# ZenHKD/ocr-vi-invoice

Hardware: AMD Instinct MI355X
Metric: invoice images/sec end-to-end (det+rec) (higher is better)
Workload: dtype f16x2

## Files before the change

### include/ocrvi.h

```cpp
#ifndef OCRVI_H
#define OCRVI_H

#include <stddef.h>
#include <stdint.h>

#ifdef __cplusplus
extern "C" {
#endif

#define OCRVI_OK 0
#define OCRVI_EINVAL (-1)
#define OCRVI_EHIP (-2)
#define OCRVI_ENOMEM (-3)
#define OCRVI_EBLOB (-4)
#define OCRVI_ERANGE (-5)

typedef enum { OCRVI_F32 = 0, OCRVI_BF16 = 1, OCRVI_F16 = 2, OCRVI_F16X2 = 3 } ocrvi_dtype;

const char* ocrvi_last_error(void);
int ocrvi_abi_version(void);

typedef struct ocrvi_det ocrvi_det;

typedef struct {
// ... 137 lines not shown

#define OCRVI_DB_TARGET_GT 0
#define OCRVI_DB_TARGET_MASK 1
#define OCRVI_DB_TARGET_THRESH 2
#define OCRVI_DB_TARGET_JOB 8
#define OCRVI_DB_TARGET_MAX_SIDE 16384
int ocrvi_db_target_jobs(const int32_t* sizes, const float* xy, const int32_t* poly_offsets, const int32_t* image_offsets, int n_images,
                         double shrink_ratio, int want_thresh, int32_t* jobs, int cap_jobs, int32_t* points, int cap_points, int32_t* n_jobs,
                         int32_t* n_points, int32_t* overflow, int threads);
int ocrvi_db_target_maps(int device, const int32_t* jobs, int n_jobs, const int32_t* points, int n_points, const int32_t* rows, int n, int S,
                         float thresh_max, float* gt, float* mask, float* thresh_map, float* thresh_mask, void* stream);
int ocrvi_resize_normalize_pad_pages(int device, const int64_t* pages, const int32_t* rows, int n, int S, float* out, void* stream);

#define OCRVI_DET_EVAL_RECORD_BYTES 104
#define OCRVI_DET_EVAL_TP 0
#define OCRVI_DET_EVAL_FP 1
#define OCRVI_DET_EVAL_FN 2
#define OCRVI_DET_EVAL_POSITIVES 3
#define OCRVI_DET_EVAL_NEGATIVES 4
#define OCRVI_DET_EVAL_K 5
#define OCRVI_DET_EVAL_POS_BCE 6
#define OCRVI_DET_EVAL_TOPK_BCE 7
#define OCRVI_DET_EVAL_DICE_INTER 8
#define OCRVI_DET_EVAL_PRED_MASK 9
#define OCRVI_DET_EVAL_GT_MASK 10
#define OCRVI_DET_EVAL_L1_NUM 11
#define OCRVI_DET_EVAL_THRESH_MASK 12
int ocrvi_det_eval_workspace_bytes(int N, int H, int W, size_t* bytes);
int ocrvi_det_eval(int device, const float* binary, const float* thresh, const float* thresh_binary, const float* bin_logits,
                   const float* gt, const float* mask, const float* thresh_map, const float* thresh_mask, int N, int H, int W,
                   double negative_ratio, void* record, void* workspace, size_t workspace_bytes, void* stream);

#define OCRVI_CTC_LOSS_MAX_TARGET 1024
int ocrvi_ctc_loss(int device, const float* log_probs, int T, int B, int C, const int32_t* targets, int Lmax, const int32_t* target_lengths,
                   const int32_t* input_lengths, int blank, double* nll, void* stream);

#define OCRVI_EDIT_DISTANCE_MAX_LEN 2048
int ocrvi_edit_distance(int device, const int32_t* pred_ids, int T, const int32_t* pred_lens, const int32_t* gt_ids, int G,
                        const int32_t* gt_lens, int B, int32_t* dist, void* stream);

int ocrvi_test_offset_conv(int device, int dtype, const float* x, const float* weight_host, const float* bias_host, int N, int C, int H, int W,
                           int stride, float* out, int iters, float* avg_ms);
int ocrvi_test_deform_conv(int device, int dtype, const float* x, const float* offset, const float* mask,
                           const float* weight_host, const float* bias_host, int N, int C, int H, int W, int Co,
                           int stride, int relu, float* out, int iters, float* avg_ms);
int ocrvi_test_deform_conv_res(int device, int dtype, const float* x, const float* offset, const float* mask,
                               const float* weight_host, const float* bias_host, const float* res, int N, int C, int H, int W, int Co,
                               int stride, int relu, float* out, int iters, float* avg_ms);
int ocrvi_test_conv(int device, int dtype, const float* x, const float* weight_host, const float* bias_host,
                    int N, int C, int H, int W, int Co, int ksize, int sh, int sw, int groups, int act, float* out,
                    int iters, float* avg_ms);
int ocrvi_test_conv_res(int device, int dtype, const float* x, const float* weight_host, const float* bias_host, const float* res, int N,
                        int C, int H, int W, int Co, int ksize, int res_mode, int act, float* out, int iters, float* avg_ms);
int ocrvi_test_bneck_tail(int device, const float* t1, const float* identity, const float* w2_host, const float* b2_host,
                          const float* w3_host, const float* b3_host, const float* w1_host, const float* b1_host, int N, int H, int W,
                          int no_phase_c, float* y_out, float* t1n_out, int iters, float* avg_ms);
int ocrvi_test_db_tail(int device, int dtype, const float* x, const float* dc1_w_bin_host, const float* dc1_b_bin_host,
                       const float* dc1_w_thr_host, const float* dc1_b_thr_host, const float* dc2_w_bin_host, const float* dc2_b_bin_host,
                       const float* dc2_w_thr_host, const float* dc2_b_thr_host, int N, int OH, int OW, int groups, int binary_only,
                       float* out, float* out2, int iters, float* avg_ms);
int ocrvi_test_gemm(int device, int dtype, const float* a, const float* weight_host, const float* bias_host, const float* res, int M,
                    int K, int N, int act, int res_post, int out_f32, float* out, int iters, float* avg_ms);
int ocrvi_test_gemm_raw(int device, int dtype, const float* a, const float* weight_host, const float* bias_host, const float* res, int M,
                        int K, int N, int act, int res_post, int out_f32, void* out_raw, float* out);
int ocrvi_test_ring_plan(int dtype, int amode, int M, int K, int N, int out_f32, int has_res, int n_cu, int32_t plan[8]);
int ocrvi_test_stem_pool(int device, int dtype, const float* x, const float* weight_host, const float* bias_host, int N, int H, int W, int fused,
                         float* out, int iters, float* avg_ms);
int ocrvi_test_attention(int device, int dtype, const float* qkv, int B, int N, int heads, float* out, int iters,
                         float* avg_ms);

int ocrvi_test_mlp(int device, int dtype, float* x, const float* ln_g_host, const float* ln_b_host, const float* w1_host, const float* b1_host,
                   const float* w2_host, const float* b2_host, const float* next_g_host, const float* next_b_host, int want_xn, int M, int D,
                   float* xn_out, int iters, float* avg_ms);
int ocrvi_test_mlp_raw(int device, int dtype, float* x, const float* ln_g_host, const float* ln_b_host, const float* w1_host, const float* b1_host,
                       const float* w2_host, const float* b2_host, const float* next_g_host, const float* next_b_host, int M, int D, void* xn_raw,
                       float* xn_out, int iters, float* avg_ms);
int ocrvi_test_pack_f16x2(const float* src, size_t n, void* dst, float* wscale);

int ocrvi_test_layernorm(int device, int dtype, const float* x, int x_f32, int out_f32, const float* gamma_host, const float* beta_host,
                         int rows, int D, float* out);
int ocrvi_test_frm_vertical(int device, int dtype, const float* kv, const float* vq_host, int B, int H, int W, int D, float* out);
int ocrvi_test_asf(int device, int dtype, const float* p2, const float* p3, const float* p4, const float* p5, const float* w_host,
                   const float* b_host, int N, int H, int W, float* out);
int ocrvi_test_maxpool(int device, int dtype, const float* x, int N, int C, int H, int W, float* out);
int ocrvi_test_db_maps(int device, const float* bin_logits, const float* thresh_logits, float k, float* binary, float* thresh,
                       float* thresh_binary, size_t n);
int ocrvi_test_ctc_logsoftmax(int device, const float* logits, int ld, int B, int T, int C, float* log_probs, int32_t* argmax_ids);

int ocrvi_prof_enable(int on);
int ocrvi_prof_reset(void);
int ocrvi_prof_report(char* buf, size_t cap);

#ifdef __cplusplus
}
#endif
#endif
```

### ocr_vi_invoice_amd/_lib.py

```python
from __future__ import annotations

import ctypes as C
import os
from typing import Optional

_HERE = os.path.dirname(os.path.abspath(__file__))
LIB_PATH = os.environ.get("OCRVI_LIB") or os.path.join(_HERE, "lib", "libocrvi.so")

OCRVI_F32, OCRVI_BF16, OCRVI_F16, OCRVI_F16X2 = 0, 1, 2, 3
DTYPES = {"f32": OCRVI_F32, "fp32": OCRVI_F32, "float32": OCRVI_F32, "bf16": OCRVI_BF16, "bfloat16": OCRVI_BF16,
          "f16": OCRVI_F16, "fp16": OCRVI_F16, "float16": OCRVI_F16,
          "f16x2": OCRVI_F16X2}
ABI_VERSION = 5

EXPORTS = [
    "ocrvi_last_error", "ocrvi_abi_version",
    "ocrvi_det_create", "ocrvi_det_destroy", "ocrvi_det_workspace_bytes", "ocrvi_det_forward", "ocrvi_det_debug_features",
    "ocrvi_rec_create", "ocrvi_rec_destroy", "ocrvi_rec_workspace_bytes", "ocrvi_rec_forward", "ocrvi_rec_debug_features",
    "ocrvi_ctc_greedy", "ocrvi_normalize_u8", "ocrvi_resize_u8", "ocrvi_crop_resize_normalize", "ocrvi_db_postprocess", "ocrvi_db_boxes_batch",
    "ocrvi_unclip_polygon", "ocrvi_db_components_workspace_bytes", "ocrvi_db_components", "ocrvi_db_boxes_batch_sparse",
    "ocrvi_test_deform_conv", "ocrvi_test_offset_conv", "ocrvi_test_conv", "ocrvi_test_gemm", "ocrvi_test_attention", "ocrvi_test_mlp", "ocrvi_test_stem_pool", "ocrvi_test_pack_f16x2",
    "ocrvi_prof_enable", "ocrvi_prof_reset", "ocrvi_prof_report",
    "ocrvi_det_status", "ocrvi_rec_status", "ocrvi_range_reset", "ocrvi_range_flag",
    "ocrvi_resize_normalize_pages", "ocrvi_crop_resize_normalize_pages", "ocrvi_db_boxes_pages",
    "ocrvi_det_binary_workspace_bytes", "ocrvi_det_forward_binary",
    "ocrvi_four_point_transform", "ocrvi_warp_perspective_u8", "ocrvi_warp_perspective_pages",
    "ocrvi_test_layernorm", "ocrvi_test_frm_vertical", "ocrvi_test_asf", "ocrvi_test_maxpool", "ocrvi_test_db_maps", "ocrvi_test_ctc_logsoftmax",
    "ocrvi_det_eval_workspace_bytes", "ocrvi_det_eval", "ocrvi_ctc_loss", "ocrvi_edit_distance",
    "ocrvi_test_deform_conv_res",
    "ocrvi_enhance_init", "ocrvi_enhance_tables", "ocrvi_enhance_workspace_bytes", "ocrvi_enhance_u8",
    "ocrvi_rgb_to_lab_u8", "ocrvi_lab_to_rgb_u8", "ocrvi_clahe_lab_u8", "ocrvi_nlm_lab_u8", "ocrvi_sharpen_u8",
    "ocrvi_min_area_quads", "ocrvi_quad_crops", "ocrvi_crop_quad_resize_normalize_pages", "ocrvi_crop_quad_resize_normalize",
    "ocrvi_jpeg_info", "ocrvi_jpeg_parse", "ocrvi_jpeg_table_entry", "ocrvi_jpeg_decode_pages",
    "ocrvi_test_conv_res", "ocrvi_test_db_tail",
    "ocrvi_db_target_jobs", "ocrvi_db_target_maps", "ocrvi_resize_normalize_pad_pages",
    "ocrvi_test_mlp_raw",
    "ocrvi_test_bneck_tail",
    "ocrvi_jpeg_quant_tables", "ocrvi_jpeg_encode_header", "ocrvi_jpeg_encode_sizes", "ocrvi_jpeg_encode_table_entry", "ocrvi_jpeg_encode_pages",
    "ocrvi_test_gemm_raw", "ocrvi_test_ring_plan",
]
PAGE_ENTRY = 4
DET_EVAL_RECORD_BYTES = 104
DET_EVAL_INT_SLOTS = ("tp", "fp", "fn", "positive_count", "negatives", "negative_count")
DET_EVAL_F64_SLOTS = ("pos_bce", "topk_bce", "dice_inter", "pred_mask", "gt_mask", "l1_num", "thresh_mask")
CTC_LOSS_MAX_TARGET = 1024
EDIT_DISTANCE_MAX_LEN = 2048
CLAHE_WORKSPACE_BYTES = 16384
ENHANCE_MIN_SIDE = 16
DB_TARGET_GT, DB_TARGET_MASK, DB_TARGET_THRESH = 0, 1, 2
DB_TARGET_JOB = 8
DB_TARGET_MAX_SIDE = 16384
JPEG_ENTRY = 64
JPEG_ENC_ENTRY = 64
JPEG_HEADER_MAX = 640


class DetCfg(C.Structure):
    _fields_ = [("dtype", C.c_int32), ("k", C.c_float), ("max_batch", C.c_int32), ("backbone", C.c_int32), ("no_dcn", C.c_int32),
                ("reserved", C.c_int32 * 3)]


class RecCfg(C.Structure):
    _fields_ = [("dtype", C.c_int32), ("dims", C.c_int32 * 3), ("num_blocks", C.c_int32 * 3), ("num_local", C.c_int32 * 3),
                ("num_classes", C.c_int32), ("blank_id", C.c_int32), ("reserved", C.c_int32 * 4)]


class JpegInfo(C.Structure):
    _fields_ = [("width", C.c_int32), ("height", C.c_int32), ("components", C.c_int32), ("h_samp", C.c_int32 * 3), ("v_samp", C.c_int32 * 3),
                ("restart_interval", C.c_int32), ("orientation", C.c_int32), ("out_height", C.c_int32), ("out_width", C.c_int32),
                ("reserved", C.c_int32), ("blocks", C.c_int64), ("stream_bytes", C.c_uint64), ("workspace_bytes", C.c_uint64),
                ("quant", (C.c_uint16 * 64) * 3), ("reason", C.c_char * 160)]


_lib: Optional[C.CDLL] = None


def load() -> C.CDLL:
    global _lib
    if _lib is not None:
        return _lib
    if not os.path.exists(LIB_PATH):
        raise RuntimeError(
            f"libocrvi.so not found at {LIB_PATH}: build it with `python -c 'import __graft_entry__ as g; g.build()'` "
            "(or `make -C ocr_vi_invoice_amd/csrc`).  There is no CPU fallback for the product path.")
    import torch
    lib = C.CDLL(LIB_PATH)
    vp, i32, f32p, i32p, sz = C.c_void_p, C.c_int, C.c_void_p, C.c_void_p, C.c_size_t
    lib.ocrvi_last_error.restype = C.c_char_p
    lib.ocrvi_last_error.argtypes = []
    lib.ocrvi_abi_version.restype = i32
    lib.ocrvi_det_create.argtypes = [i32, vp, sz, C.POINTER(DetCfg), C.POINTER(vp)]
    lib.ocrvi_det_destroy.argtypes = [vp]
    lib.ocrvi_det_destroy.restype = None
    lib.ocrvi_det_workspace_bytes.argtypes = [vp, i32, i32, i32, C.POINTER(sz)]
    lib.ocrvi_det_forward.argtypes = [vp, f32p, i32, i32, i32, f32p, f32p, f32p, f32p, f32p, vp, sz, vp]
    lib.ocrvi_det_binary_workspace_bytes.argtypes = [vp, i32, i32, i32, C.POINTER(sz)]
    lib.ocrvi_det_forward_binary.argtypes = [vp, f32p, i32, i32, i32, f32p, vp, sz, vp]
    lib.ocrvi_det_debug_features.argtypes = [vp, i32, i32, i32, f32p, f32p, f32p, f32p, f32p, vp, sz, vp]
    lib.ocrvi_rec_create.argtypes = [i32, vp, sz, C.POINTER(RecCfg), C.POINTER(vp)]
    lib.ocrvi_rec_destroy.argtypes = [vp]
    lib.ocrvi_rec_destroy.restype = None
    lib.ocrvi_rec_workspace_bytes.argtypes = [vp, i32, i32, i32, C.POINTER(sz)]
    lib.ocrvi_rec_forward.argtypes = [vp, f32p, i32, i32, i32, f32p, i32p, i32p, i32p, vp, sz, vp]
    lib.ocrvi_rec_debug_features.argtypes = [vp, i32, i32, i32, f32p, f32p, vp, sz, vp]
    lib.ocrvi_ctc_greedy.argtypes = [i32, f32p, i32, i32, i32, i32, i32p, i32p, i32p, vp]
    lib.ocrvi_normalize_u8.argtypes = [i32, vp, i32, i32, i32, f32p, vp]
    lib.ocrvi_resize_u8.argtypes = [i32, vp, i32, i32, vp, i32, i32, vp]
    lib.ocrvi_crop_resize_normalize.argtypes = [i32, vp, i32, i32, i32, i32p, i32, i32, i32, f32p, vp]
    lib.ocrvi_db_postprocess.argtypes = [vp, i32, i32, C.c_float, C.c_float, i32, C.c_float, C.c_float, vp, i32, vp, vp, i32, C.POINTER(i32)]
    lib.ocrvi_db_components_workspace_bytes.argtypes = [i32, i32, i32]
    lib.ocrvi_db_components_workspace_bytes.restype = sz
    lib.ocrvi_db_components.argtypes = [i32, vp, i32, i32, i32, C.c_float, vp, vp, vp, i32, vp, vp, C.c_longlong, vp, vp]
    lib.ocrvi_db_boxes_batch_sparse.argtypes = [vp, vp, vp, i32, vp, vp, C.c_longlong, i32, i32, i32, C.c_float, i32, C.c_float, C.c_float,
                                                C.c_double, C.c_double, i32, i32, i32, vp, vp, i32, vp, i32, vp]
    lib.ocrvi_unclip_polygon.argtypes = [vp, i32, C.c_double, vp, i32, C.POINTER(i32)]
    lib.ocrvi_db_boxes_batch.argtypes = [vp, i32, i32, i32, C.c_float, C.c_float, i32, C.c_float, C.c_float, C.c_double, C.c_double, i32, i32, i32,
                                         vp, vp, i32, vp, i32]
    lib.ocrvi_resize_normalize_pages.argtypes = [i32, vp, i32, i32, i32, f32p, vp]
    lib.ocrvi_crop_resize_normalize_pages.argtypes = [i32, vp, i32, i32p, i32, i32, i32, f32p, vp]
    lib.ocrvi_four_point_transform.argtypes = [vp, vp, vp, i32p, i32p]
    lib.ocrvi_warp_perspective_u8.argtypes = [i32, vp, i32, i32, vp, vp, i32, i32, vp]
    lib.ocrvi_warp_perspective_pages.argtypes = [i32, vp, vp, vp, i32, vp]
    lib.ocrvi_db_boxes_pages.argtypes = [vp, i32, i32, i32, C.c_float, C.c_float, i32, C.c_float, C.c_float, vp, vp, vp, vp, vp,
                                         vp, i32, vp, vp, vp, i32, vp, vp, i32]
    lib.ocrvi_test_deform_conv.argtypes = [i32, i32, f32p, f32p, f32p, vp, vp, i32, i32, i32, i32, i32, i32, i32, f32p, i32,
                                           C.POINTER(C.c_float)]
    lib.ocrvi_test_deform_conv_res.argtypes = [i32, i32, f32p, f32p, f32p, vp, vp, f32p, i32, i32, i32, i32, i32, i32, i32, f32p, i32,
                                               C.POINTER(C.c_float)]
    lib.ocrvi_test_offset_conv.argtypes = [i32, i32, f32p, vp, vp, i32, i32, i32, i32, i32, f32p, i32, C.POINTER(C.c_float)]
    lib.ocrvi_test_conv.argtypes = [i32, i32, f32p, vp, vp, i32, i32, i32, i32, i32, i32, i32, i32, i32, i32, f32p, i32,
                                    C.POINTER(C.c_float)]
    lib.ocrvi_test_conv_res.argtypes = [i32, i32, f32p, vp, vp, f32p, i32, i32, i32, i32, i32, i32, i32, i32, f32p, i32, C.POINTER(C.c_float)]
    lib.ocrvi_test_bneck_tail.argtypes = [i32, f32p, f32p, vp, vp, vp, vp, vp, vp, i32, i32, i32, i32, f32p, f32p, i32, C.POINTER(C.c_float)]
    lib.ocrvi_test_db_tail.argtypes = [i32, i32, f32p, vp, vp, vp, vp, vp, vp, vp, vp, i32, i32, i32, i32, i32, f32p, f32p, i32,
                                       C.POINTER(C.c_float)]
    lib.ocrvi_test_gemm.argtypes = [i32, i32, f32p, vp, vp, f32p, i32, i32, i32, i32, i32, i32, f32p, i32, C.POINTER(C.c_float)]
    lib.ocrvi_test_gemm_raw.argtypes = [i32, i32, f32p, vp, vp, f32p, i32, i32, i32, i32, i32, i32, vp, f32p]
    lib.ocrvi_test_ring_plan.argtypes = [i32, i32, i32, i32, i32, i32, i32, i32, C.POINTER(C.c_int32)]
    lib.ocrvi_test_stem_pool.argtypes = [i32, i32, f32p, vp, vp, i32, i32, i32, i32, f32p, i32, C.POINTER(C.c_float)]
    lib.ocrvi_test_attention.argtypes = [i32, i32, f32p, i32, i32, i32, f32p, i32, C.POINTER(C.c_float)]
    lib.ocrvi_test_mlp.argtypes = [i32, i32, f32p, vp, vp, vp, vp, vp, vp, vp, vp, i32, i32, i32, f32p, i32, C.POINTER(C.c_float)]
    lib.ocrvi_test_mlp_raw.argtypes = [i32, i32, f32p, vp, vp, vp, vp, vp, vp, vp, vp, i32, i32, vp, f32p, i32, C.POINTER(C.c_float)]
    lib.ocrvi_test_pack_f16x2.argtypes = [f32p, sz, vp, C.POINTER(C.c_float)]
    lib.ocrvi_test_layernorm.argtypes = [i32, i32, f32p, i32, i32, vp, vp, i32, i32, f32p]
    lib.ocrvi_test_frm_vertical.argtypes = [i32, i32, f32p, vp, i32, i32, i32, i32, f32p]
    lib.ocrvi_test_asf.argtypes = [i32, i32, f32p, f32p, f32p, f32p, vp, vp, i32, i32, i32, f32p]
    lib.ocrvi_test_maxpool.argtypes = [i32, i32, f32p, i32, i32, i32, i32, f32p]
    lib.ocrvi_test_db_maps.argtypes = [i32, f32p, f32p, C.c_float, f32p, f32p, f32p, sz]
    lib.ocrvi_test_ctc_logsoftmax.argtypes = [i32, f32p, i32, i32, i32, i32, f32p, i32p]
    lib.ocrvi_det_eval_workspace_bytes.argtypes = [i32, i32, i32, C.POINTER(sz)]
    lib.ocrvi_det_eval.argtypes = [i32, f32p, f32p, f32p, f32p, f32p, f32p, f32p, f32p, i32, i32, i32, C.c_double, vp, vp, sz, vp]
    lib.ocrvi_ctc_loss.argtypes = [i32, f32p, i32, i32, i32, i32p, i32, i32p, i32p, i32, vp, vp]
    lib.ocrvi_edit_distance.argtypes = [i32, i32p, i32, i32p, i32p, i32, i32p, i32, i32p, vp]
    lib.ocrvi_enhance_init.argtypes = [i32]
    lib.ocrvi_enhance_tables.argtypes = [vp, sz, C.POINTER(sz)]
    lib.ocrvi_enhance_workspace_bytes.argtypes = [i32, i32, C.POINTER(sz)]
    lib.ocrvi_enhance_u8.argtypes = [i32, vp, i32, i32, vp, vp, sz, vp]
    for name in ("ocrvi_rgb_to_lab_u8", "ocrvi_lab_to_rgb_u8", "ocrvi_nlm_lab_u8", "ocrvi_sharpen_u8"):
        getattr(lib, name).argtypes = [i32, vp, i32, i32, vp, vp]
    lib.ocrvi_clahe_lab_u8.argtypes = [i32, vp, i32, i32, vp, vp, sz, vp]
    lib.ocrvi_min_area_quads.argtypes = [vp, vp, i32, vp, vp]
    lib.ocrvi_quad_crops.argtypes = [vp, vp, i32, vp, vp, vp, vp]
    lib.ocrvi_crop_quad_resize_normalize_pages.argtypes = [i32, vp, i32, i32p, vp, i32, i32, i32, f32p, vp]
    lib.ocrvi_crop_quad_resize_normalize.argtypes = [i32, vp, i32, i32, i32, i32p, vp, i32, i32, i32, f32p, vp]
    lib.ocrvi_jpeg_info.argtypes = [vp, sz, C.POINTER(JpegInfo)]
    lib.ocrvi_jpeg_parse.argtypes = [vp, sz, vp, sz, C.POINTER(sz)]
    lib.ocrvi_jpeg_table_entry.argtypes = [C.POINTER(JpegInfo), sz, C.c_int64, C.c_int64, C.c_int64, C.c_int64, vp]
    lib.ocrvi_jpeg_decode_pages.argtypes = [i32, vp, vp, i32, vp, vp, sz, vp]
    lib.ocrvi_jpeg_quant_tables.argtypes = [i32, vp, vp]
    lib.ocrvi_jpeg_encode_header.argtypes = [i32, i32, i32, i32, i32, vp, sz, C.POINTER(sz)]
    lib.ocrvi_jpeg_encode_sizes.argtypes = [i32, i32, i32, i32, C.POINTER(C.c_int64), C.POINTER(C.c_uint64), C.POINTER(C.c_uint64), vp]
    lib.ocrvi_jpeg_encode_table_entry.argtypes = [i32, i32, i32, i32, i32, C.c_int64, C.c_int64, C.c_int64, C.c_int64, C.c_int64, vp]
    lib.ocrvi_jpeg_encode_pages.argtypes = [i32, vp, vp, i32, vp, vp, vp, sz, vp]
    lib.ocrvi_db_target_jobs.argtypes = [vp, vp, vp, vp, i32, C.c_double, i32, vp, i32, vp, i32, C.POINTER(C.c_int32), C.POINTER(C.c_int32),
                                         C.POINTER(C.c_int32), i32]
    lib.ocrvi_db_target_maps.argtypes = [i32, vp, i32, vp, i32, vp, i32, i32, C.c_float, f32p, f32p, f32p, f32p, vp]
    lib.ocrvi_resize_normalize_pad_pages.argtypes = [i32, vp, vp, i32, i32, f32p, vp]
    lib.ocrvi_det_status.argtypes = [vp]
    lib.ocrvi_rec_status.argtypes = [vp]
    lib.ocrvi_range_reset.argtypes = [i32, vp]
    lib.ocrvi_range_flag.argtypes = [i32, C.POINTER(i32)]
    lib.ocrvi_prof_enable.argtypes = [i32]
    lib.ocrvi_prof_reset.argtypes = []
    lib.ocrvi_prof_report.argtypes = [C.c_char_p, sz]
    for name in EXPORTS:
# ... 45 lines not shown
```

### ocr_vi_invoice_amd/csrc/conv_launch.h

```cpp
#pragma once
#include <stdlib.h>
#include <string.h>

#include <algorithm>

#include "conv_gemm.h"
#include "gemm_ring.h"
#include "gconv32.h"
#include "dcn_pipe.h"
#include "offs_conv.h"
#include "conv3_halo.h"

namespace ocrvi {

template <typename T, int AMODE, int BM, int BN, int WM, int WN>
static int launch_tile(const ConvParams& p, hipStream_t stream) {
    constexpr int smem = (BM + BN) * 128;
    const int total = cdiv(p.M, BM) * (p.Np / BN);
    hipLaunchKernelGGL((conv_gemm_kernel<T, AMODE, BM, BN, WM, WN, 0>), dim3(total, p.groups), dim3(256), smem, stream, p);
    OCRVI_HIP(hipGetLastError());
    return OCRVI_OK;
}

template <typename T, int BM, int NW, int SPS, bool F32O, bool C3, int BN, int ACT>
// ... 140 lines not shown
    }
}

template <typename T>
int launch_conv(const ConvParams& p_in, int amode, hipStream_t stream) {
    constexpr int EPC = TypeInfo<T>::EPC, BKE = 8 * EPC;
    ConvParams p = p_in;
    OCRVI_CHECK(p.M > 0 && p.M < (1 << 23) && p.OW > 0 && p.OH > 0, OCRVI_EINVAL, "conv: M=%d outside (0, 2^23)", p.M);
    p.mg_ow = ((1ull << 40) / (unsigned long long)p.OW) + 1;
    p.mg_oh = ((1ull << 40) / (unsigned long long)p.OH) + 1;
    p.identity_pix = (amode == AM_CONV1 && p.SH == 1 && p.SW == 1 && p.PH == 0 && p.PW == 0 && p.H == p.OH && p.W == p.OW &&
                      p.store_mode == ST_NHWC && p.res_mode != RES_UP2) ? 1 : 0;
    {
        const int osz = (p.out_f32 || sizeof(T) == 4) ? 4 : 2, per = 16 / osz;
        p.epi_lds = (p.store_mode == ST_NHWC && p.res_mode != RES_UP2 && p.N_g % per == 0 && p.ldo % per == 0 &&
                     p.out_coff % per == 0 && ((uintptr_t)p.out & 15) == 0) ? 1 : 0;
        const bool raw32 = IsF32<T>::value || (p.out_f32 && p.res_f32);
        p.res_in_store = (p.epi_lds && p.res_mode == RES_SAME && osz == 4 && raw32 && p.act == ACT_NONE &&
                          p.ldr % 4 == 0 && ((uintptr_t)p.res & 15) == 0) ? 1 : 0;
    }
    OCRVI_CHECK(p.x && p.w && p.out, OCRVI_EINVAL, "conv: null operand");
    OCRVI_CHECK(p.M > 0 && p.M == p.n_img * p.OH * p.OW, OCRVI_EINVAL, "conv: M=%d != %d*%d*%d", p.M, p.n_img, p.OH, p.OW);
    OCRVI_CHECK(p.Kp > 0 && p.Kp % BKE == 0, OCRVI_EINVAL, "conv: Kp=%d not a multiple of %d", p.Kp, BKE);
    OCRVI_CHECK(p.groups >= 1 && p.N_g >= 1, OCRVI_EINVAL, "conv: bad groups/N");
    OCRVI_CHECK((size_t)p.M * (size_t)(p.ldo > 32 ? p.ldo : 32) < ((size_t)1 << 40), OCRVI_EINVAL, "conv: output too large");
    if (p.store_mode == ST_DB_TAIL) {
        OCRVI_CHECK(amode == AM_CONV1 && p.shuffle_co == 64 && p.N_g == 256 && p.Np == 256 && p.out2 && p.offs && p.bias && p.groups == 2,
                    OCRVI_EINVAL, "db-tail deconv: needs 2 groups of 4x64 columns, both logit maps and the second-deconv weights");
    } else if (p.store_mode == ST_DB_BIN) {
        OCRVI_CHECK(amode == AM_CONV1 && p.shuffle_co == 64 && p.N_g == 256 && p.Np == 256 && p.offs && p.bias && p.groups == 1 && p.out_f32,
                    OCRVI_EINVAL, "db-bin deconv: needs one group of 4x64 columns, the fp32 binary map and the second-deconv weights");
    } else if (p.store_mode != ST_DCN_OFFS) {
        OCRVI_CHECK(p.N_g % 4 == 0 && p.ldo % 4 == 0 && p.out_coff % 4 == 0, OCRVI_EINVAL,
                    "conv: N_g=%d ldo=%d coff=%d must be multiples of 4", p.N_g, p.ldo, p.out_coff);
    } else {
        OCRVI_CHECK(p.bias && p.N_g <= 32 && p.groups == 1, OCRVI_EINVAL, "dcn offset conv: needs bias, N<=32");
    }
    if (p.res_mode != RES_NONE) OCRVI_CHECK(p.res && p.ldr % 4 == 0, OCRVI_EINVAL, "conv: residual missing / ldr%%4");
    if (p.res_mode == RES_UP2) OCRVI_CHECK(p.OH % 2 == 0 && p.OW % 2 == 0, OCRVI_EINVAL, "conv: RES_UP2 needs even OH/OW");
    if (p.store_mode == ST_SHUFFLE2)
        OCRVI_CHECK(p.shuffle_co > 0 && p.shuffle_co % 4 == 0 && p.N_g == 4 * p.shuffle_co, OCRVI_EINVAL, "conv: bad pixel-shuffle N");
    if (amode == AM_ROWS) {
        OCRVI_CHECK(p.groups == 1 && p.Hp >= (p.OH - 1) * p.SH + p.KH && p.Wp >= (p.OW - 1) * p.SW + 8 && p.Wp % 2 == 0 &&
                        p.Kp >= p.KH * 32 && (p.SW * 4) % EPC == 0,
                    OCRVI_EINVAL, "rows-mode conv: padded input %dx%d too small for %dx%d out", p.Hp, p.Wp, p.OH, p.OW);
        return launch_mode<T, AM_ROWS>(p, stream);
    }
    OCRVI_CHECK(p.Cin_g % EPC == 0 && p.Cin % EPC == 0 && p.cin_off % EPC == 0 && p.cin_off + p.groups * p.Cin_g <= p.Cin,
                OCRVI_EINVAL, "conv: channel counts Cin=%d Cin_g=%d off=%d must be multiples of %d", p.Cin, p.Cin_g, p.cin_off, EPC);
    const int ks = amode == AM_CONV1 ? 1 : 3;
    OCRVI_CHECK(p.Kp >= ks * ks * p.Cin_g, OCRVI_EINVAL, "conv: Kp=%d < %d", p.Kp, ks * ks * p.Cin_g);
    OCRVI_CHECK((p.OH - 1) * p.SH - p.PH + ks - 1 < p.H + ks && (p.OW - 1) * p.SW - p.PW + ks - 1 < p.W + ks, OCRVI_EINVAL,
                "conv: output %dx%d inconsistent with input %dx%d", p.OH, p.OW, p.H, p.W);
    if constexpr (sizeof(T) == 2) {
        if (gconv32_eligible(p, amode, 2)) return launch_gconv32<T>(p, stream);
    }
    if (offs_conv_eligible(p, amode, TypeInfo<T>::dtype)) return launch_offs_conv<T>(p, stream);
    if constexpr (IsSplit<T>::value) {
        if (conv3_halo_eligible(p, amode, TypeInfo<T>::dtype)) return launch_conv3_halo<T>(p, stream);
    }
    OCRVI_CHECK(!p.w_quartets, OCRVI_EINVAL,
                "conv3x3: weights are packed for the halo kernel but this call is not eligible for it (stride / epilogue / alignment)");
    if (gemm_ring_eligible(p, amode, TypeInfo<T>::dtype)) return launch_gemm_ring<T>(p, amode, stream);
    switch (amode) {
        case AM_CONV1: return launch_mode<T, AM_CONV1>(p, stream);
        case AM_CONV3: return launch_mode<T, AM_CONV3>(p, stream);
        case AM_DCN:
            OCRVI_CHECK(p.offs && p.Cin_g % BKE == 0 && p.groups == 1, OCRVI_EINVAL, "dcn: needs offsets and Cin %% %d == 0", BKE);
            if (dcn_pipe_eligible(p, TypeInfo<T>::dtype)) return launch_dcn_pipe<T>(p, stream);
            OCRVI_CHECK(!dcn_pipe_packing(TypeInfo<T>::dtype, p.Cin_g), OCRVI_EINVAL,
                        "dcn: weights are packed for the pipelined kernel but this call is not eligible for it (epilogue / alignment)");
            return launch_mode<T, AM_DCN>(p, stream);
        default: break;
    }
    set_error("conv: unknown A mode %d", amode);
    return OCRVI_EINVAL;
}

}
```

### ocr_vi_invoice_amd/csrc/gconv32.h

```cpp
#pragma once
#include "conv_gemm.h"

namespace ocrvi {

constexpr int GC_PS = 96;
constexpr int GC_TH = 4;
constexpr int GC_NBX = 5;

template <typename T, bool F32O>
__global__ __launch_bounds__(256, 2) void gconv32_kernel(const ConvParams p, int TH, int nbx, int bands_y, int bands_x, unsigned hw_magic) {
    constexpr int PS = GC_PS, MB = (GC_TH * GC_NBX + 3) / 4;
    extern __shared__ __attribute__((aligned(16))) char smem[];
    const int tid = threadIdx.x, lane = tid & 63, wave = tid >> 6;
    const int lr = lane & 15, g4 = lane >> 4;
    const int TW = 16 * nbx, HW = TW + 2, HH = TH + 2;
    char* const halo = smem;
    char* const wl = smem + HH * HW * PS;
    const int gp = blockIdx.y;
    const int ntile = p.n_img * bands_y * bands_x;
    const T* const Xg = (const T*)p.x + p.cin_off + gp * 32;
    constexpr int HPASS = ((GC_TH + 2) * (16 * GC_NBX + 2) * 4 + 255) / 256, WPASS = (32 * 36 + 255) / 256;
    uint4 hv[HPASS];
    const int htotal = HH * HW * 4;
    auto tile_origin = [&](int t, int& img, int& y0, int& x0) {
        const int bx = t % bands_x;
        t /= bands_x;
        const int by = t % bands_y;
        img = t / bands_y;
        y0 = by * TH;
        x0 = bx * TW;
    };
    auto fetch = [&](int t) {
        int img, y0, x0;
        tile_origin(t, img, y0, x0);
        const T* X = Xg + (size_t)img * p.H * p.W * p.Cin;
#pragma unroll
        for (int k = 0; k < HPASS; ++k) {
            const int i = min(tid + 256 * k, htotal - 1);
            const int pix = i >> 2, c = i & 3;
            const int hy = (int)(((unsigned)pix * hw_magic) >> 16), hx = pix - hy * HW;
            const int iy = min(max(y0 + hy - 1, 0), p.H - 1), ix = min(max(x0 + hx - 1, 0), p.W - 1);
            hv[k] = *(const uint4*)(X + ((size_t)iy * p.W + ix) * p.Cin + c * 8);
        }
    };
    auto stage = [&](int t) {
        int img, y0, x0;
        tile_origin(t, img, y0, x0);
#pragma unroll
        for (int k = 0; k < HPASS; ++k) {
            const int i = tid + 256 * k;
            if (i < htotal) {
                const int pix = i >> 2, c = i & 3;
                const int hy = (int)(((unsigned)pix * hw_magic) >> 16), hx = pix - hy * HW;
                const int iy = y0 + hy - 1, ix = x0 + hx - 1;
// ... 61 lines not shown
            const int r = tap / 3, s = tap - r * 3;
            uint4 wf[2];
#pragma unroll
            for (int nb = 0; nb < 2; ++nb) wf[nb] = *(const uint4*)(wl + (tap * 32 + wrow[nb]) * PS + g4 * 16);
#pragma unroll
            for (int m = 0; m < MB; ++m) {
                if (wave + 4 * m < nblk) {
                    const uint4 xf = *(const uint4*)(halo + aoff[m] + (r * HW + s) * PS);
                    Mma<T>::half(wf[0], xf, acc[m][0]);
                    Mma<T>::half(wf[1], xf, acc[m][1]);
                }
            }
        }
        __syncthreads();
        if (next < ntile) stage(next);
        int img, y0, x0;
        tile_origin(tile, img, y0, x0);
#pragma unroll
        for (int m = 0; m < MB; ++m) {
            const int mb = wave + 4 * m, ty = mb / nbx, tb = mb - ty * nbx;
            const int y = y0 + ty, x = x0 + tb * 16 + lr;
            if (mb >= nblk || y >= p.H || x >= p.W) continue;
            const size_t pix = ((size_t)img * p.H + y) * p.W + x;
            float v[2][4];
#pragma unroll
            for (int nb = 0; nb < 2; ++nb) {
                const int ch = gp * 32 + (F32O ? nb * 16 + 4 * g4 : 8 * g4 + 4 * nb);
                v[nb][0] = acc[m][nb][0] + bias_r[nb].x; v[nb][1] = acc[m][nb][1] + bias_r[nb].y;
                v[nb][2] = acc[m][nb][2] + bias_r[nb].z; v[nb][3] = acc[m][nb][3] + bias_r[nb].w;
                if (p.res_post) activate(v[nb]);
                if (F32O && p.res_mode == RES_SAME) {
                    const float4 rv = *(const float4*)((const float*)p.res + pix * p.ldr + ch);
                    v[nb][0] += rv.x; v[nb][1] += rv.y; v[nb][2] += rv.z; v[nb][3] += rv.w;
                }
                if (!p.res_post) activate(v[nb]);
                if (F32O) *(float4*)((float*)p.out + pix * p.ldo + p.out_coff + ch) = make_float4(v[nb][0], v[nb][1], v[nb][2], v[nb][3]);
            }
            if (!F32O) {
                union { T e[8]; uint4 u; } pk;
#pragma unroll
                for (int e = 0; e < 4; ++e) {
                    pk.e[e] = from_f32<T>(v[0][e]);
                    pk.e[4 + e] = from_f32<T>(v[1][e]);
                }
                *(uint4*)((T*)p.out + pix * p.ldo + p.out_coff + gp * 32 + 8 * g4) = pk.u;
            }
        }
        if (next >= ntile) break;
        tile = next;
        __syncthreads();
    }
}

static inline bool gconv32_eligible(const ConvParams& p, int amode, int esz) {
    static const bool on = !(getenv("OCRVI_GCONV32") && atoi(getenv("OCRVI_GCONV32")) == 0);
    if (!on || amode != AM_CONV3 || esz != 2 || p.groups < 2 || p.Cin_g != 32 || p.N_g != 32 || p.KH != 3) return false;
    if (p.SH != 1 || p.SW != 1 || p.PH != 1 || p.PW != 1 || p.H != p.OH || p.W != p.OW || p.store_mode != ST_NHWC) return false;
    if (p.Kp < 288 || p.Cin % 8 != 0 || p.cin_off % 8 != 0 || ((uintptr_t)p.x & 15) != 0 || ((uintptr_t)p.w & 15) != 0 || p.Kp % 8 != 0) return false;
    const int og = p.out_f32 ? 4 : 8;
    if (p.ldo % og != 0 || p.out_coff % og != 0 || ((uintptr_t)p.out & 15) != 0) return false;
    if (p.res_mode == RES_SAME) return p.out_f32 && p.res_f32 && p.ldr % 4 == 0 && ((uintptr_t)p.res & 15) == 0;
    return p.res_mode == RES_NONE;
}

template <typename T>
static int launch_gconv32(const ConvParams& p, hipStream_t stream) {
    const int nbx = std::min(GC_NBX, cdiv(p.W, 16));
    const int th = p.H % 4 == 0 ? 4 : (p.H % 3 == 0 ? 3 : (p.H < 4 ? p.H : 4));
    const int bands_x = cdiv(p.W, 16 * nbx), bands_y = cdiv(p.H, th);
    const int smem = (th + 2) * (16 * nbx + 2) * GC_PS + 9 * 32 * GC_PS;
    const unsigned hw_magic = 65536u / (unsigned)(16 * nbx + 2) + 1;
    int n_cu = 0;
    OCRVI_TRY(device_cus(&n_cu));
    const int ntile = p.n_img * bands_y * bands_x;
    const int per_group = std::max(1, 2 * n_cu / p.groups);
    const dim3 grid(cdiv(ntile, cdiv(ntile, per_group)), p.groups);
    if (p.out_f32) {
        auto k = gconv32_kernel<T, true>;
        OCRVI_TRY(ensure_max_smem((const void*)k, 80 * 1024));
        hipLaunchKernelGGL(k, grid, dim3(256), smem, stream, p, th, nbx, bands_y, bands_x, hw_magic);
    } else {
        auto k = gconv32_kernel<T, false>;
        OCRVI_TRY(ensure_max_smem((const void*)k, 80 * 1024));
        hipLaunchKernelGGL(k, grid, dim3(256), smem, stream, p, th, nbx, bands_y, bands_x, hw_magic);
    }
    OCRVI_HIP(hipGetLastError());
    return OCRVI_OK;
}

}
```

### ocr_vi_invoice_amd/csrc/host_util.hip

```cpp
#include <stdarg.h>
#include <stdlib.h>
#include <string.h>

#include <math.h>

#include <algorithm>
#include <map>
#include <mutex>

#include "conv_gemm.h"
#include "gemm_ring.h"
#include "dcn_pipe.h"

namespace ocrvi {

static thread_local char g_err[512] = "";
void set_error(const char* fmt, ...) {
    va_list ap;
    va_start(ap, fmt);
    vsnprintf(g_err, sizeof(g_err), fmt, ap);
    va_end(ap);
}
const char* last_error_cstr() { return g_err; }

#pragma pack(push, 1)
struct BlobEntry {
    char name[64];
    uint32_t ndim;
    uint32_t dims[4];
    uint64_t offset;
    uint64_t count;
};
#pragma pack(pop)
static_assert(sizeof(BlobEntry) == 100, "entry layout");

int Blob::parse(const void* blob, size_t bytes) {
    OCRVI_CHECK(blob && bytes >= 16 && memcmp(blob, "OCRVIW1\0", 8) == 0, OCRVI_EBLOB, "weight blob: bad magic / too short");
    uint32_t n;
    memcpy(&n, (const char*)blob + 8, 4);
    OCRVI_CHECK(16 + (size_t)n * sizeof(BlobEntry) <= bytes, OCRVI_EBLOB, "weight blob: truncated table");
    tensors.resize(n);
    for (uint32_t i = 0; i < n; ++i) {
        BlobEntry e;
        memcpy(&e, (const char*)blob + 16 + (size_t)i * sizeof(BlobEntry), sizeof(e));
        e.name[63] = 0;
        OCRVI_CHECK(e.ndim <= 4 && e.offset % 4 == 0 && e.offset + e.count * 4 <= bytes, OCRVI_EBLOB,
                    "weight blob: tensor %s out of bounds", e.name);
        size_t prod = 1;
        for (uint32_t d = 0; d < e.ndim; ++d) prod *= e.dims[d];
        OCRVI_CHECK(prod == e.count, OCRVI_EBLOB, "weight blob: tensor %s count mismatch", e.name);
        BlobTensor& t = tensors[i];
        t.name = e.name;
        t.ndim = (int)e.ndim;
        for (int d = 0; d < 4; ++d) t.dims[d] = d < (int)e.ndim ? (int)e.dims[d] : 1;
        t.data = (const float*)((const char*)blob + e.offset);
        t.count = e.count;
    }
    return OCRVI_OK;
}
const BlobTensor* Blob::find(const std::string& name) const {
    for (const auto& t : tensors)
        if (t.name == name) return &t;
    return nullptr;
}
int Blob::get(const std::string& name, int d0, int d1, int d2, int d3, const BlobTensor** out) const {
// ... 320 lines not shown
int RangeWatch::snapshot(hipStream_t s) {
    if (!dev_word) return OCRVI_OK;
    OCRVI_HIP(hipMemcpyAsync(host_word, dev_word, sizeof(unsigned), hipMemcpyDeviceToHost, s));
    return OCRVI_OK;
}
int RangeWatch::status(const char* what) const {
    OCRVI_CHECK(!host_word || *(volatile unsigned*)host_word == 0, OCRVI_ERANGE,
                "%s: an f16x2 activation left fp16's range (|x| >= 65520) on this device since the last ocrvi_range_reset: the results of that "
                "forward are not valid -- run this model with dtype f32 (or f16x2 after rescaling the offending layer)", what);
    return OCRVI_OK;
}
RangeWatch::~RangeWatch() {
    if (host_word) (void)hipHostFree(host_word);
}
extern "C" int ocrvi_range_reset(int device, void* stream) {
    DeviceGuard dg(device);
    OCRVI_HIP(dg.err);
    unsigned* w = nullptr;
    OCRVI_TRY(range_flag_bind(&w));
    OCRVI_HIP(hipMemsetAsync(w, 0, sizeof(unsigned), (hipStream_t)stream));
    return OCRVI_OK;
}
extern "C" int ocrvi_range_flag(int device, int* raised) {
    OCRVI_CHECK(raised, OCRVI_EINVAL, "range_flag: null out");
    DeviceGuard dg(device);
    OCRVI_HIP(dg.err);
    unsigned* w = nullptr;
    unsigned v = 0;
    OCRVI_TRY(range_flag_bind(&w));
    OCRVI_HIP(hipDeviceSynchronize());
    OCRVI_HIP(hipMemcpy(&v, w, sizeof(v), hipMemcpyDeviceToHost));
    *raised = v != 0;
    return OCRVI_OK;
}

int launch_conv_dt(int dtype, const ConvParams& p, int amode, hipStream_t stream) {
    char tag[160];
    double flops = 0, bytes = 0;
    if (g_prof_on) {
        const int ks = amode == AM_CONV1 ? 1 : (amode == AM_ROWS ? p.KH : 3);
        const double kvalid = amode == AM_ROWS ? (double)p.KH * p.KH * 3 : (double)ks * ks * p.Cin_g;
        const double esz = (double)dtype_size(dtype);
        flops = 2.0 * p.M * p.N_g * p.groups * kvalid;
        bytes = (double)p.n_img * p.H * p.W * (amode == AM_ROWS ? 4 : p.Cin_g * p.groups) * esz + (double)p.N_g * p.groups * kvalid * esz +
                (double)p.M * p.N_g * p.groups * (p.out_f32 ? 4.0 : esz) + (p.res ? (double)p.M * p.N_g * p.groups * (p.res_f32 ? 4.0 : esz) : 0.0) +
                (p.offs ? (double)p.M * 27 * 4 : 0.0);
        ConvParams q = p;
        q.identity_pix = (amode == AM_CONV1 && p.SH == 1 && p.SW == 1 && p.PH == 0 && p.PW == 0 && p.H == p.OH && p.W == p.OW &&
                          p.store_mode == ST_NHWC && p.res_mode != RES_UP2) ? 1 : 0;
        const bool ring = gemm_ring_eligible(q, amode, dtype);
        const bool pipe = amode == AM_DCN && dcn_pipe_eligible(q, dtype);
        static const bool detail = getenv("OCRVI_PROF_DETAIL") != nullptr;
        const bool halo = conv3_halo_eligible(q, amode, dtype);
        if (halo && !detail)
            snprintf(tag, sizeof(tag), "conv3x3_halo_%s", dtype_name(dtype));
        else if (halo)
            snprintf(tag, sizeof(tag), "conv3x3_halo_%s M%d N%d K%d g%d s%d", dtype_name(dtype), p.M, p.N_g, (int)kvalid, p.groups, p.SH);
        else if (ring && !detail)
            snprintf(tag, sizeof(tag), "gemm_ring_%s", dtype_name(dtype));
        else if (pipe && !detail)
            snprintf(tag, sizeof(tag), "dcn3x3_pipe128x%d_%s", p.Np % 256 == 0 ? 256 : 128, dtype_name(dtype));
        else if (pipe)
            snprintf(tag, sizeof(tag), "dcn3x3_pipe128x%d_%s M%d N%d K%d g%d s%d", p.Np % 256 == 0 ? 256 : 128, dtype_name(dtype), p.M, p.N_g, (int)kvalid,
                     p.groups, p.SH);
        else if (detail)
            snprintf(tag, sizeof(tag), "%s%s_%dx%d_%s M%d N%d K%d g%d s%d", ring ? "ring_" : "", amode_name(amode, p), amode == AM_DCN ? 64 : 128, (amode == AM_DCN && p.Np % 256 == 0) ? 256 : conv_bn_for(p.N_g), dtype_name(dtype), p.M,
                     p.N_g, (int)kvalid, p.groups, p.SH);
        else
            snprintf(tag, sizeof(tag), "%s%s_%dx%d_%s", ring ? "ring_" : "", amode_name(amode, p), amode == AM_DCN ? 64 : 128, (amode == AM_DCN && p.Np % 256 == 0) ? 256 : conv_bn_for(p.N_g), dtype_name(dtype));
    }
    ProfScope ps(tag, flops, bytes, stream);
    switch (dtype) {
        case OCRVI_F32: return launch_conv<float>(p, amode, stream);
        case OCRVI_BF16: return launch_conv<bf16_t>(p, amode, stream);
        case OCRVI_F16: return launch_conv<f16_t>(p, amode, stream);
        case OCRVI_F16X2: return launch_conv<f16x2_t>(p, amode, stream);
    }
    set_error("unknown dtype %d", dtype);
    return OCRVI_EINVAL;
}

}

extern "C" int ocrvi_prof_enable(int on) {
    std::lock_guard<std::mutex> lk(ocrvi::g_prof_mu);
    ocrvi::g_prof_on = on != 0;
    return OCRVI_OK;
}
extern "C" int ocrvi_prof_reset(void) {
    std::lock_guard<std::mutex> lk(ocrvi::g_prof_mu);
    for (auto& e : ocrvi::g_prof) { (void)hipEventDestroy(e.e0); (void)hipEventDestroy(e.e1); }
    ocrvi::g_prof.clear();
    return OCRVI_OK;
}
extern "C" int ocrvi_prof_report(char* buf, size_t cap) {
    using namespace ocrvi;
    OCRVI_CHECK(buf && cap > 2, OCRVI_EINVAL, "prof_report: null buffer");
    std::lock_guard<std::mutex> lk(g_prof_mu);
    struct Agg { double ms = 0, flops = 0, bytes = 0; long n = 0; };
    std::map<std::string, Agg> agg;
    for (auto& e : g_prof) {
        OCRVI_HIP(hipEventSynchronize(e.e1));
        float ms = 0.f;
        OCRVI_HIP(hipEventElapsedTime(&ms, e.e0, e.e1));
        Agg& a = agg[e.tag];
        a.ms += ms; a.flops += e.flops; a.bytes += e.bytes; a.n += 1;
    }
// ... 28 lines not shown
```

Measured before the change: 326.6.

## Add f16x2 halo-tiled grouped 3x3 conv kernel for 32-channel groups

```diff
diff --git a/include/ocrvi.h b/include/ocrvi.h
--- a/include/ocrvi.h
+++ b/include/ocrvi.h
@@ -213,6 +213,8 @@
                     int iters, float* avg_ms);
 int ocrvi_test_conv_res(int device, int dtype, const float* x, const float* weight_host, const float* bias_host, const float* res, int N,
                         int C, int H, int W, int Co, int ksize, int res_mode, int act, float* out, int iters, float* avg_ms);
+int ocrvi_test_gconv_res(int device, int dtype, const float* x, const float* weight_host, const float* bias_host, const float* res, int N,
+                         int C, int H, int W, int Co, int groups, int act, int res_post, float* out, int iters, float* avg_ms);
 int ocrvi_test_bneck_tail(int device, const float* t1, const float* identity, const float* w2_host, const float* b2_host,
                           const float* w3_host, const float* b3_host, const float* w1_host, const float* b1_host, int N, int H, int W,
                           int no_phase_c, float* y_out, float* t1n_out, int iters, float* avg_ms);
diff --git a/ocr_vi_invoice_amd/_lib.py b/ocr_vi_invoice_amd/_lib.py
--- a/ocr_vi_invoice_amd/_lib.py
+++ b/ocr_vi_invoice_amd/_lib.py
@@ -38,6 +38,7 @@
     "ocrvi_test_bneck_tail",
     "ocrvi_jpeg_quant_tables", "ocrvi_jpeg_encode_header", "ocrvi_jpeg_encode_sizes", "ocrvi_jpeg_encode_table_entry", "ocrvi_jpeg_encode_pages",
     "ocrvi_test_gemm_raw", "ocrvi_test_ring_plan",
+    "ocrvi_test_gconv_res",
 ]
 PAGE_ENTRY = 4
 DET_EVAL_RECORD_BYTES = 104
@@ -131,6 +132,7 @@
     lib.ocrvi_test_conv.argtypes = [i32, i32, f32p, vp, vp, i32, i32, i32, i32, i32, i32, i32, i32, i32, i32, f32p, i32,
                                     C.POINTER(C.c_float)]
     lib.ocrvi_test_conv_res.argtypes = [i32, i32, f32p, vp, vp, f32p, i32, i32, i32, i32, i32, i32, i32, i32, f32p, i32, C.POINTER(C.c_float)]
+    lib.ocrvi_test_gconv_res.argtypes = [i32, i32, f32p, vp, vp, f32p, i32, i32, i32, i32, i32, i32, i32, i32, f32p, i32, C.POINTER(C.c_float)]
     lib.ocrvi_test_bneck_tail.argtypes = [i32, f32p, f32p, vp, vp, vp, vp, vp, vp, i32, i32, i32, i32, f32p, f32p, i32, C.POINTER(C.c_float)]
     lib.ocrvi_test_db_tail.argtypes = [i32, i32, f32p, vp, vp, vp, vp, vp, vp, vp, vp, i32, i32, i32, i32, i32, f32p, f32p, i32,
                                        C.POINTER(C.c_float)]
diff --git a/ocr_vi_invoice_amd/csrc/conv_launch.h b/ocr_vi_invoice_amd/csrc/conv_launch.h
--- a/ocr_vi_invoice_amd/csrc/conv_launch.h
+++ b/ocr_vi_invoice_amd/csrc/conv_launch.h
@@ -216,8 +216,8 @@
     OCRVI_CHECK(p.Kp >= ks * ks * p.Cin_g, OCRVI_EINVAL, "conv: Kp=%d < %d", p.Kp, ks * ks * p.Cin_g);
     OCRVI_CHECK((p.OH - 1) * p.SH - p.PH + ks - 1 < p.H + ks && (p.OW - 1) * p.SW - p.PW + ks - 1 < p.W + ks, OCRVI_EINVAL,
                 "conv: output %dx%d inconsistent with input %dx%d", p.OH, p.OW, p.H, p.W);
-    if constexpr (sizeof(T) == 2) {
-        if (gconv32_eligible(p, amode, 2)) return launch_gconv32<T>(p, stream);
+    if constexpr (sizeof(T) == 2 || IsSplit<T>::value) {
+        if (gconv32_eligible(p, amode, (int)sizeof(T))) return launch_gconv32<T>(p, stream);
     }
     if (offs_conv_eligible(p, amode, TypeInfo<T>::dtype)) return launch_offs_conv<T>(p, stream);
     if constexpr (IsSplit<T>::value) {
diff --git a/ocr_vi_invoice_amd/csrc/gconv32.h b/ocr_vi_invoice_amd/csrc/gconv32.h
--- a/ocr_vi_invoice_amd/csrc/gconv32.h
+++ b/ocr_vi_invoice_amd/csrc/gconv32.h
@@ -1,5 +1,6 @@
 #pragma once
 #include "conv_gemm.h"
+#include "conv3_halo.h"
 
 namespace ocrvi {
 
@@ -167,40 +168,254 @@
     }
 }
 
+constexpr int GX_PS = 128;
+
+template <typename T, bool F32O>
+__global__ __launch_bounds__(512) void gconv32x2_kernel(const ConvParams p, int TH, int nbx, int bands_y, int bands_x, unsigned hw_magic) {
+    static_assert(IsSplit<T>::value, "the f16x2 form");
+    constexpr int PS = GX_PS, MB = (GC_TH * GC_NBX + 7) / 8;
+    typedef typename Mma<T>::u4v U;
+    extern __shared__ __attribute__((aligned(16))) char smem[];
+    const int tid = threadIdx.x, lane = tid & 63;
+    const int wave = __builtin_amdgcn_readfirstlane(tid >> 6);
+    const int lr = lane & 15, g4 = lane >> 4;
+    const int TW = 16 * nbx, HW = TW + 2, HH = TH + 2;
+    char* const halo = smem;
+    char* const wl = smem + HH * HW * PS;
+    const int gp = blockIdx.y;
+    const int ntile = p.n_img * bands_y * bands_x;
+    const char* const Xg = (const char*)p.x + ((size_t)p.cin_off + gp * 32) * 4;
+    const size_t pix_b = (size_t)p.Cin * 4;
+    constexpr int HPASS = ((GC_TH + 2) * (16 * GC_NBX + 2) * 4 + 511) / 512, WPASS = (32 * 36 + 511) / 512;
+    uint4 hv[HPASS][2];
+    const int htotal = HH * HW * 4;
+    auto tile_origin = [&](int t, int& img, int& y0, int& x0) {
+        const int bx = t % bands_x;
+        t /= bands_x;
+        const int by = t % bands_y;
+        img = t / bands_y;
+        y0 = by * TH;
+        x0 = bx * TW;
+    };
+    auto fetch = [&](int t) {
+        int img, y0, x0;
+        tile_origin(t, img, y0, x0);
+        const char* X = Xg + (size_t)img * p.H * p.W * pix_b;
+#pragma unroll
+        for (int k = 0; k < HPASS; ++k) {
+            const int i = min(tid + 512 * k, htotal - 1);
+            const int pix = i >> 2, j = i & 3;
+            const int hy = (int)(((unsigned)pix * hw_magic) >> 16), hx = pix - hy * HW;
+            const int iy = min(max(y0 + hy - 1, 0), p.H - 1), ix = min(max(x0 + hx - 1, 0), p.W - 1);
+            const char* src = X + ((size_t)iy * p.W + ix) * pix_b + j * 32;
+            hv[k][0] = *(const uint4*)src;
+            hv[k][1] = *(const uint4*)(src + 16);
+        }
+    };
+    auto put_units = [&](char* row, int ridx, int j, const uint4& c0, const uint4& c1, bool live) {
+        U H, L;
+        Mma<T>::regroup(c0, c1, H, L);
+        if (!live) H = L = (U){0u, 0u, 0u, 0u};
+        const int sw = swz_halo(ridx);
+        *(U*)(row + (((2 * j) ^ sw) << 4)) = H;
+        *(U*)(row + (((2 * j + 1) ^ sw) << 4)) = L;
+    };
+    auto stage = [&](int t) {
+        int img, y0, x0;
+        tile_origin(t, img, y0, x0);
+#pragma unroll
+        for (int k = 0; k < HPASS; ++k) {
+            const int i = tid + 512 * k;
+            if (i < htotal) {
+                const int pix = i >> 2, j = i & 3;
+                const int hy = (int)(((unsigned)pix * hw_magic) >> 16), hx = pix - hy * HW;
+                const int iy = y0 + hy - 1, ix = x0 + hx - 1;
+                const bool in = (unsigned)iy < (unsigned)p.H && (unsigned)ix < (unsigned)p.W;
+                put_units(halo + pix * PS, pix, j, hv[k][0], hv[k][1], in);
+            }
+        }
+    };
+    int tile = blockIdx.x;
+    if (tile >= ntile) return;
+    fetch(tile);
+    {
+        const char* Wg = (const char*)p.w + (size_t)gp * p.Np * p.Kp * 4;
+        uint4 wv[WPASS][2];
+#pragma unroll
+        for (int k = 0; k < WPASS; ++k) {
+            const int i = min(tid + 512 * k, 32 * 36 - 1);
+            const int n = i / 36, rem = i - n * 36, tap = rem >> 2, j = rem & 3;
+            const char* src = Wg + ((size_t)n * p.Kp + tap * 32) * 4 + j * 32;
+            wv[k][0] = *(const uint4*)src;
+            wv[k][1] = *(const uint4*)(src + 16);
+        }
+#pragma unroll
+        for (int k = 0; k < WPASS; ++k) {
+            const int i = tid + 512 * k;
+            if (i < 32 * 36) {
+                const int n = i / 36, rem = i - n * 36, tap = rem >> 2, j = rem & 3;
+                put_units(wl + (tap * 32 + n) * PS, n, j, wv[k][0], wv[k][1], true);
+            }
+        }
+    }
+    stage(tile);
+    __syncthreads();
+    const int nblk = TH * nbx;
+    bool live[MB];
+    int bty[MB], btb[MB], apix[MB];
+#pragma unroll
+    for (int m = 0; m < MB; ++m) {
+        const int mb = wave + 8 * m;
+        live[m] = mb < nblk;
+        bty[m] = live[m] ? mb / nbx : 0;
+        btb[m] = live[m] ? mb - bty[m] * nbx : 0;
+        apix[m] = bty[m] * HW + btb[m] * 16 + lr;
+    }
+    int woff[2];
+#pragma unroll
+    for (int h = 0; h < 2; ++h) woff[h] = lr * PS + (((2 * g4 + h) ^ swz_halo(lr)) << 4);
+    float4 bias_r[2];
+#pragma unroll
+    for (int nb = 0; nb < 2; ++nb) {
+        const int ch = gp * 32 + nb * 16 + 4 * g4;
+        bias_r[nb] = p.bias ? *(const float4*)(p.bias + ch) : make_float4(0.f, 0.f, 0.f, 0.f);
+    }
+    auto activate = [&](float (&v)[4]) {
+        if (p.act == ACT_RELU) {
+#pragma unroll
+            for (int e = 0; e < 4; ++e) v[e] = fmaxf(v[e], 0.f);
+        } else if (p.act == ACT_GELU) {
+#pragma unroll
+            for (int e = 0; e < 4; ++e) v[e] = gelu_erf(v[e]);
+        }
+    };
+    struct Frag { U wH[2], wL[2], xH[MB], xL[MB]; };
+    auto read_frags = [&](int tap, Frag& f) {
+        const int r = tap / 3, s = tap - r * 3;
+#pragma unroll
+        for (int nb = 0; nb < 2; ++nb) {
+            f.wH[nb] = *(const U*)(wl + (tap * 32 + nb * 16) * PS + woff[0]);
+            f.wL[nb] = *(const U*)(wl + (tap * 32 + nb * 16) * PS + woff[1]);
+        }
+        const int d = r * HW + s;
+#pragma unroll
+        for (int m = 0; m < MB; ++m) {
+            const int q = apix[m] + d;
+            const int a = q * PS + (((2 * g4) ^ swz_halo(q)) << 4);
+            f.xH[m] = *(const U*)(halo + a);
+            f.xL[m] = *(const U*)(halo + (a ^ 16));
+        }
+    };
+    int next = tile + gridDim.x;
+    if (next < ntile) fetch(next);
+    for (;;) {
+        f32x4 acc[MB][2];
+#pragma unroll
+        for (int m = 0; m < MB; ++m) acc[m][0] = acc[m][1] = (f32x4){0.f, 0.f, 0.f, 0.f};
+        Frag fr[2];
+        read_frags(0, fr[0]);
+#pragma unroll
+        for (int tap = 0; tap < 9; ++tap) {
+            if (tap + 1 < 9) read_frags(tap + 1, fr[(tap + 1) & 1]);
+            __builtin_amdgcn_sched_barrier(0);
+            const Frag& f = fr[tap & 1];
+#pragma unroll
+            for (int m = 0; m < MB; ++m) {
+                if (live[m]) {
+                    Mma<T>::three(f.wH[0], f.wL[0], f.xH[m], f.xL[m], acc[m][0]);
+                    Mma<T>::three(f.wH[1], f.wL[1], f.xH[m], f.xL[m], acc[m][1]);
+                }
+            }
+            __builtin_amdgcn_sched_barrier(0);
+        }
+        __syncthreads();
+        if (next < ntile) stage(next);
+        const int next2 = next + gridDim.x;
+        if (!F32O && next2 < ntile) fetch(next2);
+        int img, y0, x0;
+        tile_origin(tile, img, y0, x0);
+        unsigned long long bad = 0;
+#pragma unroll
+        for (int m = 0; m < MB; ++m) {
+            const int y = y0 + bty[m], x = x0 + btb[m] * 16 + lr;
+            const bool ok = live[m] && y < p.H && x < p.W;
+            const size_t pix = ((size_t)img * p.H + y) * p.W + x;
+            float v[2][4];
+#pragma unroll
+            for (int nb = 0; nb < 2; ++nb) {
+                const int ch = gp * 32 + nb * 16 + 4 * g4;
+                v[nb][0] = unscale<T>(acc[m][nb][0], p.wscale) + bias_r[nb].x; v[nb][1] = unscale<T>(acc[m][nb][1], p.wscale) + bias_r[nb].y;
+                v[nb][2] = unscale<T>(acc[m][nb][2], p.wscale) + bias_r[nb].z; v[nb][3] = unscale<T>(acc[m][nb][3], p.wscale) + bias_r[nb].w;
+                if (p.res_post) activate(v[nb]);
+                if (F32O && p.res_mode == RES_SAME && ok) {
+                    const float4 rv = *(const float4*)((const float*)p.res + pix * p.ldr + ch);
+                    v[nb][0] += rv.x; v[nb][1] += rv.y; v[nb][2] += rv.z; v[nb][3] += rv.w;
+                }
+                if (!p.res_post) activate(v[nb]);
+                if (!F32O) bad |= f16x2_out_of_range(v[nb]) & __builtin_amdgcn_ballot_w64(ok);
+            }
+            if (ok) {
+                char* const o = (char*)p.out + (pix * p.ldo + p.out_coff + gp * 32 + 4 * g4) * 4;
+                if (F32O) {
+                    *(float4*)o = make_float4(v[0][0], v[0][1], v[0][2], v[0][3]);
+                    *(float4*)(o + 64) = make_float4(v[1][0], v[1][1], v[1][2], v[1][3]);
+                } else {
+                    *(uint4*)o = Chunk<T>::pack(v[0]);
+                    *(uint4*)(o + 64) = Chunk<T>::pack(v[1]);
+                }
+            }
+        }
+        if (!F32O) f16x2_raise(bad);
+        if (F32O && next2 < ntile) fetch(next2);
+        if (next >= ntile) break;
+        tile = next;
+        next = next2;
+        __syncthreads();
+    }
+}
+
 static inline bool gconv32_eligible(const ConvParams& p, int amode, int esz) {
     static const bool on = !(getenv("OCRVI_GCONV32") && atoi(getenv("OCRVI_GCONV32")) == 0);
-    if (!on || amode != AM_CONV3 || esz != 2 || p.groups < 2 || p.Cin_g != 32 || p.N_g != 32 || p.KH != 3) return false;
-    if (p.SH != 1 || p.SW != 1 || p.PH != 1 || p.PW != 1 || p.H != p.OH || p.W != p.OW || p.store_mode != ST_NHWC) return false;
-    if (p.Kp < 288 || p.Cin % 8 != 0 || p.cin_off % 8 != 0 || ((uintptr_t)p.x & 15) != 0 || ((uintptr_t)p.w & 15) != 0 || p.Kp % 8 != 0) return false;
-    const int og = p.out_f32 ? 4 : 8;
+    if (!on || amode != AM_CONV3 || (esz != 2 && esz != 4) || p.groups < 2 || p.Cin_g != 32 || p.N_g != 32 || p.Np < 32 || p.KH != 3) return false;
+    if (p.SH != 1 || p.SW != 1 || p.PH != 1 || p.PW != 1 || p.H != p.OH || p.W != p.OW || p.store_mode != ST_NHWC || p.w_quartets) return false;
+    const int epc = 16 / esz;
+    if (p.Kp < 288 || p.Cin % epc != 0 || p.cin_off % epc != 0 || ((uintptr_t)p.x & 15) != 0 || ((uintptr_t)p.w & 15) != 0 || p.Kp % epc != 0) return false;
+    const int og = (p.out_f32 || esz == 4) ? 4 : 8;
     if (p.ldo % og != 0 || p.out_coff % og != 0 || ((uintptr_t)p.out & 15) != 0) return false;
-    if (p.res_mode == RES_SAME) return p.out_f32 && p.res_f32 && p.ldr % 4 == 0 && ((uintptr_t)p.res & 15) == 0;
+    if (p.res_mode == RES_SAME) return p.out_f32 && p.res_f32 && p.res && p.ldr % 4 == 0 && ((uintptr_t)p.res & 15) == 0;
     return p.res_mode == RES_NONE;
 }
 
+static inline int gconv32_tile_h(int H) { return H % 4 == 0 ? 4 : (H % 3 == 0 ? 3 : (H < 4 ? H : 4)); }
+
 template <typename T>
 static int launch_gconv32(const ConvParams& p, hipStream_t stream) {
+    constexpr bool X2 = IsSplit<T>::value;
+    constexpr int PS = X2 ? GX_PS : GC_PS, NT = X2 ? 512 : 256;
     const int nbx = std::min(GC_NBX, cdiv(p.W, 16));
-    const int th = p.H % 4 == 0 ? 4 : (p.H % 3 == 0 ? 3 : (p.H < 4 ? p.H : 4));
+    const int th = gconv32_tile_h(p.H);
     const int bands_x = cdiv(p.W, 16 * nbx), bands_y = cdiv(p.H, th);
-    const int smem = (th + 2) * (16 * nbx + 2) * GC_PS + 9 * 32 * GC_PS;
+    const int smem = (th + 2) * (16 * nbx + 2) * PS + 9 * 32 * PS;
     const unsigned hw_magic = 65536u / (unsigned)(16 * nbx + 2) + 1;
     int n_cu = 0;
     OCRVI_TRY(device_cus(&n_cu));
     const int ntile = p.n_img * bands_y * bands_x;
-    const int per_group = std::max(1, 2 * n_cu / p.groups);
+    const int per_group = std::max(1, (X2 ? 1 : 2) * n_cu / p.groups);
     const dim3 grid(cdiv(ntile, cdiv(ntile, per_group)), p.groups);
-    if (p.out_f32) {
-        auto k = gconv32_kernel<T, true>;
-        OCRVI_TRY(ensure_max_smem((const void*)k, 80 * 1024));
-        hipLaunchKernelGGL(k, grid, dim3(256), smem, stream, p, th, nbx, bands_y, bands_x, hw_magic);
+    constexpr int max_smem = (GC_TH + 2) * (16 * GC_NBX + 2) * PS + 9 * 32 * PS;
+    auto run = [&](auto k) -> int {
+        OCRVI_TRY(ensure_max_smem((const void*)k, max_smem));
+        hipLaunchKernelGGL(k, grid, dim3(NT), smem, stream, p, th, nbx, bands_y, bands_x, hw_magic);
+        OCRVI_HIP(hipGetLastError());
+        return OCRVI_OK;
+    };
+    if constexpr (X2) {
+        if (p.out_f32) return run(gconv32x2_kernel<T, true>);
+        return run(gconv32x2_kernel<T, false>);
     } else {
-        auto k = gconv32_kernel<T, false>;
-        OCRVI_TRY(ensure_max_smem((const void*)k, 80 * 1024));
-        hipLaunchKernelGGL(k, grid, dim3(256), smem, stream, p, th, nbx, bands_y, bands_x, hw_magic);
-    }
-    OCRVI_HIP(hipGetLastError());
-    return OCRVI_OK;
+        if (p.out_f32) return run(gconv32_kernel<T, true>);
+        return run(gconv32_kernel<T, false>);
+    }
 }
 
 }
diff --git a/ocr_vi_invoice_amd/csrc/host_util.hip b/ocr_vi_invoice_amd/csrc/host_util.hip
--- a/ocr_vi_invoice_amd/csrc/host_util.hip
+++ b/ocr_vi_invoice_amd/csrc/host_util.hip
@@ -11,6 +11,7 @@
 #include "conv_gemm.h"
 #include "gemm_ring.h"
 #include "dcn_pipe.h"
+#include "gconv32.h"
 
 namespace ocrvi {
 
@@ -437,7 +438,12 @@
         const bool pipe = amode == AM_DCN && dcn_pipe_eligible(q, dtype);
         static const bool detail = getenv("OCRVI_PROF_DETAIL") != nullptr;
         const bool halo = conv3_halo_eligible(q, amode, dtype);
-        if (halo && !detail)
+        const bool ghalo = dtype == OCRVI_F16X2 && gconv32_eligible(q, amode, 4);
+        if (ghalo && !detail)
+            snprintf(tag, sizeof(tag), "gconv3x3_halo_%s", dtype_name(dtype));
+        else if (ghalo)
+            snprintf(tag, sizeof(tag), "gconv3x3_halo_%s M%d N%d K%d g%d s%d", dtype_name(dtype), p.M, p.N_g, (int)kvalid, p.groups, p.SH);
+        else if (halo && !detail)
             snprintf(tag, sizeof(tag), "conv3x3_halo_%s", dtype_name(dtype));
         else if (halo)
             snprintf(tag, sizeof(tag), "conv3x3_halo_%s M%d N%d K%d g%d s%d", dtype_name(dtype), p.M, p.N_g, (int)kvalid, p.groups, p.SH);
```

Result: no change. 328.9, median of 6 (+0.7%).
